# Allenxuxu/gev

Hardware: AMD Instinct MI355X
Metric: GiB/s WS payload unmasked (device-resident) + frames/s, 64 KiB masked frames (higher is better)
Workload: dtype u8

## Files before the change

gev_amd/csrc/gevws_walk.hip:

```cpp
#include <chrono>

#include "gevws_internal.hpp"
#include "gevws_small.hpp"

namespace {

__device__ __forceinline__ void put_partial(uint64_t* part, uint32_t b, int k, uint64_t v, uint32_t tag) {
  uint64_t* p = part + 2 * ((uint64_t)b * kDecFields + k);
  put_granule(p, (uint32_t)v, tag);
  put_granule(p + 1, (uint32_t)(v >> 32), tag);
}

__device__ void scan_partials_wave(const uint64_t* __restrict__ part, uint32_t tag, uint64_t* __restrict__ blk,
                                   uint32_t nblk, uint64_t max_frames, uint64_t payload_cap,
                                   gevws_summary* __restrict__ sum) {
  constexpr int P = 4;
  const int lane = threadIdx.x & 63;
  uint64_t carry[kDecFields] = {0, 0, 0, 0, 0};
  uint32_t bad = 0;
  for (uint64_t base = 0; base < nblk; base += 64 * P) {
    const uint64_t i0 = base + (uint64_t)lane * P;
    uint64_t g[P][kDecFields][2];
#pragma unroll
    for (int r = 0; r < P; ++r)
#pragma unroll
      for (int k = 0; k < kDecFields; ++k)
#pragma unroll
        for (int h = 0; h < 2; ++h)
          g[r][k][h] = (i0 + r < nblk) ? load_granule(part + 2 * ((i0 + r) * kDecFields + k) + h) : 0;
    uint64_t loc[kDecFields] = {0, 0, 0, 0, 0};
    uint64_t loc0[P], loc1[P];
#pragma unroll
    for (int r = 0; r < P; ++r)
#pragma unroll
      for (int k = 0; k < kDecFields; ++k) {
        uint64_t v = 0;
        if (i0 + r < nblk) {
          const uint64_t* q = part + 2 * ((i0 + r) * kDecFields + k);
          v = (uint64_t)take_granule(q, g[r][k][0], tag, bad) | ((uint64_t)take_granule(q + 1, g[r][k][1], tag, bad) << 32);
        }
        loc[k] += v;
        if (k == 0) loc0[r] = v;
        if (k == 1) loc1[r] = v;
      }
    const uint64_t inc0 = wave_incl_scan(loc[0]), inc1 = wave_incl_scan(loc[1]);
    uint64_t b0 = carry[0] + inc0 - loc[0], b1 = carry[1] + inc1 - loc[1];
#pragma unroll
    for (int r = 0; r < P; ++r) {
      if (i0 + r < nblk) {
        uint64_t* q = blk + (i0 + r) * kDecFields;
        q[0] = b0;
        q[1] = b1;
        b0 += loc0[r];
        b1 += loc1[r];
      }
    }
#pragma unroll
    for (int k = 0; k < kDecFields; ++k) carry[k] += wave_sum(loc[k]);
  }
  bad = (uint32_t)wave_sum(bad);
  if (lane == 0) {
    gevws_summary sm;
    memset(&sm, 0, sizeof(sm));
    sm.frames = carry[0];
    sm.payload_bytes = carry[1];
    sm.payload_len = carry[2];
    sm.errors = carry[3] & 0xffffffffull;
    sm.flags = (carry[3] >> 32) ? GEVWS_SUMMARY_UNORDERED : 0u;
    sm.run_frames = carry[4];
    sm.status = bad ? GEVWS_ERR_DEVICE
                    : (carry[0] > max_frames || carry[1] > payload_cap) ? GEVWS_ERR_CAPACITY : GEVWS_OK;
    *sum = sm;
  }
}

__device__ __forceinline__ void walk_block_done(uint32_t* __restrict__ done, uint32_t nblk, const uint64_t* __restrict__ part,
                                                uint32_t tag, uint64_t* __restrict__ blk, uint64_t max_frames,
                                                uint64_t payload_cap, gevws_summary* __restrict__ sum, bool wrote) {
  __shared__ uint32_t s_last;
  if (wrote) __builtin_amdgcn_s_waitcnt(0);
  __syncthreads();
  if (threadIdx.x == 0)
    s_last = __hip_atomic_fetch_add(done, 1u, __ATOMIC_RELAXED, __HIP_MEMORY_SCOPE_AGENT) == nblk - 1 ? 1u : 0u;
  __syncthreads();
  if (s_last) {
    if (threadIdx.x < 64) scan_partials_wave(part, tag, blk, nblk, max_frames, payload_cap, sum);
    if (threadIdx.x == 0) __hip_atomic_store(done, 0u, __ATOMIC_RELAXED, __HIP_MEMORY_SCOPE_AGENT);
  }
}

constexpr uint64_t kWriterChainsPerCU = 128;
constexpr uint32_t kEntryGranMinShift = 6;
constexpr uint64_t kEntryBudget = 1ull << 29;
constexpr uint32_t kSlotShift = 5;
constexpr uint64_t kSlotAlign = 1ull << kSlotShift;
constexpr uint32_t kLenEsc = (1u << 21) - 1;
struct WalkEntry {
  uint32_t mask;
  uint32_t w;
};
static_assert(sizeof(WalkEntry) == 8, "one dwordx2 per entry");
__device__ __forceinline__ WalkEntry make_entry(uint32_t key, uint64_t L, uint32_t meta) {
  const uint32_t hlen = meta >> 16, masked = (meta >> 8) & 1u;
  const uint32_t ext = hlen - 2 - 4 * masked;
  const uint32_t form = ext == 0 ? 0u : (ext == 2 ? 1u : 2u);
  const uint32_t l21 = L < kLenEsc ? (uint32_t)L : kLenEsc;
  return WalkEntry{key, (meta & 0x1ffu) | (form << 9) | (l21 << 11)};
}
__device__ __forceinline__ uint32_t entry_hlen(const WalkEntry& e) {
  const uint32_t form = (e.w >> 9) & 3u;
  return 2 + (form == 2 ? 8u : 2u * form) + 4 * ((e.w >> 8) & 1u);
}
__device__ __forceinline__ uint32_t entry_len21(const WalkEntry& e) { return e.w >> 11; }

__device__ __forceinline__ bool entry_slots_of(const gevws_conn_in& ci, uint32_t c, uint64_t n_entries,
                                              uint32_t gshift, uint64_t& base, uint64_t& cap) {
  if (n_entries == 0 || ci.len >= (1ull << 32)) return false;
  base = kSlotAlign * ((ci.off >> (gshift + kSlotShift)) + (uint64_t)c);
  cap = kSlotAlign * ((ci.len >> (gshift + kSlotShift)) + 1);
  return base + cap <= n_entries;
}

__device__ __forceinline__ bool out_of_order(const gevws_conn_in* __restrict__ conns, uint32_t c,
                                             const gevws_conn_in& ci) {
  if (c == 0) return false;
  const gevws_conn_in p = conns[c - 1];
  return ci.off < p.off || ci.off - p.off < p.len;
}

__device__ __forceinline__ int walk_parse(uint64_t lo, uint64_t hi, uint64_t avail, uint32_t& meta, uint32_t& hlen,
                                          uint64_t& L, uint32_t& key) {
  const uint32_t b1 = (uint32_t)(lo >> 8) & 0xffu;
  const uint32_t masked = b1 >> 7, len7 = b1 & 0x7fu;
  const bool e16 = len7 == 126, e64 = len7 == 127;
  hlen = 2 + (e64 ? 8u : (e16 ? 2u : 0u)) + 4 * masked;
  const uint64_t L64 = __builtin_bswap64((lo >> 16) | (hi << 48));
  const uint64_t L16 = (((lo >> 16) & 0xff) << 8) | ((lo >> 24) & 0xff);
  L = e64 ? L64 : (e16 ? L16 : (uint64_t)len7);
  key = (e64 ? (uint32_t)(hi >> 16) : (e16 ? (uint32_t)(lo >> 32) : (uint32_t)(lo >> 16))) & (0u - masked);
  meta = ((uint32_t)lo & 0xffu) | (masked << 8) | (hlen << 16);
  const bool have_hdr = avail >= 6 && avail >= hlen;
  if (have_hdr && e64 && (L64 >> 63)) return GEVWS_ERR_LEN_MSB;
  return (have_hdr && avail - hlen >= L) ? GEVWS_OK : GEVWS_NEED_MORE;
}

struct WalkRes {
  uint64_t pos, nf, pb, pl, same, lastf, firstf, err;
  int32_t st;
  bool rec;
};
__device__ __forceinline__ WalkRes walk_res_fresh(uint64_t err = 0, int32_t st = GEVWS_OK) {
  WalkRes R;
  R.pos = R.nf = R.pb = R.pl = R.same = R.firstf = 0;
// ... 95 lines not shown
            qhi[0] = nhi;
            bool stop = false;
#pragma unroll
            for (int j = 0; j < D; ++j) {
              if (!stop && (uint32_t)j < qn) {
                uint32_t m2, h2, k2;
                uint64_t L2;
                const int r = walk_parse(qlo[j], qhi[j], len - pos, m2, h2, L2, k2);
                if (r != GEVWS_OK) {
                  if (r == GEVWS_ERR_LEN_MSB) { st = GEVWS_ERR_LEN_MSB; err += 1; }
                  fail = stop = true;
                } else {
                  put_entry(k2, L2, m2);
                  pos += h2 + L2;
                  if (h2 + L2 != fsz) {
                    stop = true;
                    run = 1;
                    prev_fsz = h2 + L2;
                  }
                }
              }
            }
            if (fail) break;
            load_window(s + pos, nlo, nhi);
            if (stop || qn < (uint32_t)D || pos + fsz > len) break;
          }
          if (fail) return false;
          if constexpr (ST == 0) *sink = WalkEntry{0, 0};
        }
      }
      return true;
    };
    uint64_t lo2 = 0, hi2 = 0;
    for (;;) {
      if (!step(lo, hi, lo2, hi2)) break;
      if (!step(lo2, hi2, lo, hi)) break;
    }
    R.pos = pos;
    R.nf = nf;
    R.pb = pb;
    R.pl = pl;
    R.same = same;
    R.lastf = lastf;
    R.firstf = firstf;
    R.err = err;
    R.st = st;
    R.rec = rec;
    if constexpr (ST == 2) {
      __asm__ volatile("" ::: "memory");
      lds_st(ring.head, (uint32_t)nf | kRingDone);
    }
}

template <uint32_t GROUP = kWriterGroup, uint32_t RING = kRing>
__device__ __forceinline__ void walk_ring_writer(WalkEntry* __restrict__ entries, WalkRing ring, uint64_t ebase,
                                                 uint64_t ecap) {
  static_assert(GROUP <= kSlotAlign && kSlotAlign % GROUP == 0 && RING % GROUP == 0 && GROUP % 4 == 0,
                "groups aligned by the slot runs, whole groups in the ring");
  uint32_t t = 0;
  bool fin = false;
  for (;;) {
    if (!fin) {
      const uint32_t hv = lds_ld(ring.head);
      __asm__ volatile("" ::: "memory");
      const uint32_t h = hv & ~kRingDone;
      while (h - t >= GROUP) {
        WalkEntry g[GROUP];
#pragma unroll
        for (uint32_t k = 0; k < GROUP; ++k) g[k] = ring.e[(t + k) & (RING - 1)];
        if (ebase != ~0ull && t + GROUP <= ecap) {
          u32x4* d = reinterpret_cast<u32x4*>(entries + ebase + t);
#pragma unroll
          for (uint32_t k = 0; k < GROUP / 2; ++k)
            d[k] = u32x4{g[2 * k].mask, g[2 * k].w, g[2 * k + 1].mask, g[2 * k + 1].w};
        }
        t += GROUP;
        __asm__ volatile("" ::: "memory");
        lds_st(ring.tail, t);
      }
      if (hv & kRingDone) {
        for (; t < h; ++t)
          if (ebase != ~0ull && t < ecap) entries[ebase + t] = ring.e[t & (RING - 1)];
        fin = true;
      }
    }
    if (__all(fin)) break;
    __builtin_amdgcn_s_sleep(2);
  }
}

template <int D, int ST>
__global__ __launch_bounds__(ST == 2 ? 2 * kCountBlock : kCountBlock) void k_walk_count(
    const uint8_t* __restrict__ in, const gevws_conn_in* __restrict__ conns, uint32_t n,
    gevws_conn_out* __restrict__ cout, uint64_t* __restrict__ blk, WalkEntry* __restrict__ entries, uint64_t n_entries,
    uint32_t gshift, uint32_t cpb, uint64_t in_bytes, uint32_t* __restrict__ done, uint64_t* __restrict__ part,
    uint32_t tag, uint64_t max_frames, uint64_t payload_cap, gevws_summary* __restrict__ sum) {
  __shared__ WalkEntry s_ring[ST == 2 ? kCountBlock * kRing : 1];
  __shared__ uint32_t s_head[ST == 2 ? kCountBlock : 1], s_tail[ST == 2 ? kCountBlock : 1];
  __shared__ uint64_t s_ebase[ST == 2 ? kCountBlock : 1], s_ecap[ST == 2 ? kCountBlock : 1];
  const uint32_t lane = threadIdx.x & 63;
  const bool walker = ST != 2 || threadIdx.x < 64;
  const uint32_t c = blockIdx.x * cpb + lane;
  const bool active = walker && lane < cpb && c < n;
  uint64_t nf = 0, pb = 0, pl = 0, err = 0, same = 0;
  gevws_conn_in ci = {0, 0};
  int32_t st = GEVWS_OK;
  uint64_t ebase = 0, ecap = 0;
  bool rec0 = false;
  if (active) {
    ci = conns[c];
    if (out_of_order(conns, c, ci)) err = 1ull << 32;
    if (ci.off > in_bytes || ci.len > in_bytes - ci.off) {
      ci.off = 0;
      ci.len = 0;
      st = GEVWS_ERR_INVALID;
      err += 1;
    }
    rec0 = entry_slots_of(ci, c, n_entries, gshift, ebase, ecap);
  }
  const WalkRing ring = {s_ring + lane * kRing, s_head + lane, s_tail + lane};
  if constexpr (ST == 2) {
    if (walker) {
      s_head[lane] = active ? 0u : kRingDone;
      s_tail[lane] = 0;
      s_ebase[lane] = rec0 ? ebase : ~0ull;
      s_ecap[lane] = ecap;
    }
    __syncthreads();
    if (!walker) walk_ring_writer(entries, ring, s_ebase[lane], s_ecap[lane]);
  }
  if (active) {
    WalkRes R = walk_res_fresh(err, st);
    walk_chain<D, ST>(in + ci.off, ci.len, rec0, ebase, ecap, entries, entries + n_entries + c, R, ring);
    nf = R.nf;
    pb = R.pb;
    pl = R.pl;
    err = R.err;
    same = R.same;
    gevws_conn_out o;
    o.first_frame = R.rec ? 1 : 0;
    o.consumed = R.pos;
    o.payload_base = pb;
    o.nframes = (uint32_t)nf;
    o.status = R.st;
    cout[c] = o;
  }
  const uint64_t vals[kDecFields] = {nf, pb, pl, err, same};
#pragma unroll
  for (int k = 0; k < kDecFields; ++k) {
    const uint64_t s = wave_sum(vals[k]);
    if (threadIdx.x == 0) {
      if (done) put_partial(part, blockIdx.x, k, s, tag);
      else blk[(uint64_t)blockIdx.x * kDecFields + k] = s;
    }
  }
  if (done) walk_block_done(done, gridDim.x, part, tag, blk, max_frames, payload_cap, sum, threadIdx.x == 0);
}

constexpr uint32_t kSyncWin = 256;
constexpr uint32_t kSyncRow = kSyncWin / 4 + 5;
constexpr int kSyncDepth = 5;
constexpr uint32_t kSplitAutoMaxLanes = 16;
constexpr uint64_t kSplitMinFramesPerConn = 256;
constexpr uint64_t kSplitMaxConnsPerCU = 64;
constexpr uint64_t kSplitMaxFrameBytes = 4096;

__device__ __forceinline__ bool sync_plausible1(uint32_t b0, uint32_t b1, uint32_t m0) {
  const uint32_t op = b0 & 0x0fu;
  const bool data = op <= 2, ctrl = op >= 8 && op <= 10;
  return (b0 & 0x70u) == 0 && (b1 >> 7) == m0 && (data || (ctrl && (b0 & 0x80u) && (b1 & 0x7fu) <= 125));
}

__device__ __forceinline__ uint64_t sync_frame(uint64_t lo, uint64_t hi, uint64_t rem, uint32_t m0) {
  const uint32_t b0 = (uint32_t)lo & 0xffu, b1 = (uint32_t)(lo >> 8) & 0xffu;
  if (!sync_plausible1(b0, b1, m0)) return 0;
  const uint32_t len7 = b1 & 0x7fu;
  const uint32_t hlen = 2 + (len7 == 127 ? 8u : (len7 == 126 ? 2u : 0u)) + 4 * (b1 >> 7);
  uint64_t L = len7;
  if (len7 == 126) {
    L = (((lo >> 16) & 0xff) << 8) | ((lo >> 24) & 0xff);
    if (L < 126) return 0;
  } else if (len7 == 127) {
    L = __builtin_bswap64((lo >> 16) | (hi << 48));
    if ((L >> 63) || L < 65536) return 0;
  }
  if (rem < hlen || rem - hlen < L) return 0;
  return hlen + L;
}

__device__ __forceinline__ void row_window(const uint32_t* __restrict__ row, uint32_t x, uint64_t& lo, uint64_t& hi) {
  const uint32_t k = x >> 2, e = x & 3;
  const uint32_t w0 = row[k], w1 = row[k + 1], w2 = row[k + 2], w3 = row[k + 3], w4 = row[k + 4];
  lo = (uint64_t)__builtin_amdgcn_alignbyte(w1, w0, e) | ((uint64_t)__builtin_amdgcn_alignbyte(w2, w1, e) << 32);
  hi = (uint64_t)__builtin_amdgcn_alignbyte(w3, w2, e) | ((uint64_t)__builtin_amdgcn_alignbyte(w4, w3, e) << 32);
}

__device__ __forceinline__ uint32_t sync_l1_mask4(uint32_t w, uint32_t wn, uint32_t mpat) {
  const uint32_t w1 = __builtin_amdgcn_alignbyte(wn, w, 1);
  const uint32_t bad = (w & 0x74747474u) | (w & (w >> 1) & 0x01010101u) | ((w1 ^ mpat) & 0x80808080u);
  const uint32_t z = ~(((bad & 0x7f7f7f7fu) + 0x7f7f7f7fu) | bad | 0x7f7f7f7fu);
  return ((z >> 7) & 1u) | ((z >> 14) & 2u) | ((z >> 21) & 4u) | ((z >> 28) & 8u);
}

constexpr int kSyncWindows = 4;
constexpr int kSyncMinInWindow = 1;
__device__ __forceinline__ bool sync_search(const uint8_t* __restrict__ s, uint64_t len, uint64_t t, uint64_t step,
                                            uint64_t qmax, uint32_t m0, uint32_t* __restrict__ row, uint64_t& b) {
  const uint32_t mpat = m0 ? 0x80808080u : 0u;
  for (int win = 0; win < kSyncWindows; ++win, t += step) {
    if (t + kSyncWin + 16 > len || t >= qmax) return false;
    uint32_t wv[kSyncRow - 1];
#pragma unroll
    for (uint32_t j = 0; j < (kSyncWin + 16) / 16; ++j) {
      const u32x4 v = ld16u(s + t + 16 * j);
#pragma unroll
      for (int e = 0; e < 4; ++e) wv[4 * j + e] = v[e];
    }
#pragma unroll
    for (uint32_t k = 0; k < kSyncRow - 1; ++k) row[k] = wv[k];
    row[kSyncRow - 1] = 0;
    uint64_t cm[kSyncWin / 64];
#pragma unroll
    for (uint32_t j = 0; j < kSyncWin / 64; ++j) {
      uint64_t m = 0;
#pragma unroll
      for (uint32_t k = 0; k < 16; ++k) m |= (uint64_t)sync_l1_mask4(wv[16 * j + k], wv[16 * j + k + 1], mpat) << (4 * k);
      cm[j] = m;
    }
    bool have = false;
    uint64_t q = 0, lb = 0;
    int h = 0;
#pragma unroll
    for (uint32_t j = 0; j < kSyncWin / 64; ++j) {
      uint64_t m = have ? 0 : cm[j];
      while (m) {
        uint32_t x = 64 * j + (uint32_t)__builtin_ctzll(m);
        m &= m - 1;
        uint64_t lo, hi;
        row_window(row, x, lo, hi);
        uint64_t f = sync_frame(lo, hi, len - (t + x), m0);
        if (f == 0) continue;
        int hh = 1;
        uint32_t last = x;
        while (hh < kSyncDepth && x + f < kSyncWin) {
          x += (uint32_t)f;
          row_window(row, x, lo, hi);
          f = sync_frame(lo, hi, len - (t + x), m0);
          if (f == 0) break;
          last = x;
          ++hh;
        }
        if (f == 0 || (hh < kSyncMinInWindow && t + x + f < len)) continue;
        have = true;
        q = t + x + f;
        lb = t + last;
        h = hh;
        m = 0;
      }
    }
    if (!have) continue;
    bool ok = true;
    while (h < kSyncDepth) {
      if (q >= qmax || q >= len) {
        ok = false;
        break;
      }
      uint64_t lo, hi;
      load_window(s + q, lo, hi);
      const uint64_t g = sync_frame(lo, hi, len - q, m0);
      if (g == 0) {
        ok = false;
        break;
      }
      lb = q;
      q += g;
      ++h;
    }
    if (ok && lb < qmax) {
      b = lb;
      return true;
    }
  }
  return false;
}

constexpr uint32_t kSplitRing = 32;
constexpr uint32_t kSplitGroup = 16;
constexpr uint32_t kSplitLdsWords = (kCountBlock * kSyncRow > 2 * kCountBlock * kSplitRing)
                                        ? kCountBlock * kSyncRow
                                        : 2 * kCountBlock * kSplitRing;

template <int KS, int D, int ST>
__global__ __launch_bounds__(ST == 2 ? 2 * kCountBlock : kCountBlock) void k_walk_split(const uint8_t* __restrict__ in,
                                                            const gevws_conn_in* __restrict__ conns, uint32_t n,
                                                            gevws_conn_out* __restrict__ cout,
                                                            uint64_t* __restrict__ blk,
                                                            WalkEntry* __restrict__ entries, uint64_t n_entries,
                                                            uint32_t gshift, uint32_t cpb, uint64_t in_bytes,
                                                            uint32_t* __restrict__ done,
                                                            uint64_t* __restrict__ part, uint32_t tag,
                                                            uint64_t max_frames,
                                                            uint64_t payload_cap, gevws_summary* __restrict__ sum,
                                                            gevws_conn_in* __restrict__ segs,
                                                            gevws_conn_out* __restrict__ sout,
                                                            uint8_t* __restrict__ srec,
                                                            uint64_t min_seg = kSplitMinBytes,
// ... 393 lines not shown
        pbase = o.payload_base;
        coff = ci.off;
      }
      for (uint64_t m = __ballot(lane < GL && nf > 0); m; m &= m - 1) {
        const int j = __builtin_ctzll(m);
        const uint64_t cnt = uniform64(__shfl(nf, j, 64));
        const uint64_t fj = uniform64(__shfl(ff, j, 64)), pj = uniform64(__shfl(pbase, j, 64));
        const uint64_t oj = uniform64(__shfl(coff, j, 64)), ej = uniform64(__shfl(ebase, j, 64));
        one_conn(cnt, fj, pj, oj, ej);
      }
    }
  }
  const uint64_t nthreads = (uint64_t)gridDim.x * kWalkBlock;
  for (uint64_t c = (uint64_t)blockIdx.x * kWalkBlock + threadIdx.x; c < n; c += nthreads) {
    if (rec_flags[c] && !unordered) continue;
    const gevws_conn_out o = out_of(c);
    const gevws_conn_in ci = conns[c];
    const uint8_t* s = in + ci.off;
    uint64_t pos = 0, poff = o.payload_base;
    for (uint64_t k = 0; k < o.nframes; ++k) {
      uint64_t lo, hi;
      load_window(s + pos, lo, hi);
      DevHdr h;
      parse_header(lo, hi, ci.len - pos, h);
      emit_record(frames, tile_first, o.first_frame + k, poff, ci.off + pos + h.hlen, h);
      poff += round16(h.length);
      pos += h.hlen + h.length;
    }
  }
}

template <class S>
__global__ __launch_bounds__(S::NT) void k_decode_small(const uint8_t* __restrict__ in, uint64_t in_bytes,
                                                        const gevws_conn_in* __restrict__ conns, uint32_t n,
                                                        gevws_frame* __restrict__ frames, uint64_t max_frames,
                                                        uint8_t* __restrict__ payload, uint64_t payload_cap,
                                                        gevws_conn_out* __restrict__ cout,
                                                        gevws_summary* __restrict__ sum,
                                                        uint32_t* __restrict__ done = nullptr,
                                                        uint32_t seq = 0, uint64_t* __restrict__ ticks = nullptr,
                                                        uint64_t* __restrict__ stage_buf = nullptr,
                                                        uint32_t* __restrict__ stage_done = nullptr,
                                                        uint32_t tag = 0, uint64_t* __restrict__ phase = nullptr) {
  (void)decode_small_body<S>(in, in_bytes, conns, n, frames, max_frames, payload, payload_cap, cout, sum, done, seq,
                             ticks, stage_buf, stage_done, tag, gridDim.x, blockIdx.x, gridDim.x, phase);
}

template <class S>
__global__ __launch_bounds__(S::NT) void k_decode_small_direct(DirectDecodeArgs a) {
  (void)decode_small_body<S>(a.in, a.in_bytes, a.conns, a.n, a.frames, a.max_frames, a.payload, a.payload_cap,
                             a.cout, a.sum, a.done, a.seq, a.ticks, a.stage_buf, a.stage_done, a.tag, a.nwg,
                             blockIdx.x, a.nwg, a.phase);
}

constexpr uint32_t kServiceMaxPasses = 1u << 16;
constexpr uint32_t kSvcCmd = 0, kSvcSeq = 1, kSvcArgs = 2, kSvcExit = kSvcArgs + 2 * kServiceArgs,
                   kSvcDone = kSvcExit + 1, kSvcCtlGranules = kSvcDone + 1;

template <class S>
__global__ __launch_bounds__(S::NT) void k_decode_service(ServiceBox* __restrict__ box, uint32_t gen, uint32_t req0,
                                                          uint64_t life_ticks, uint32_t* __restrict__ done,
                                                          uint64_t* __restrict__ ticks, uint64_t* __restrict__ ctl,
                                                          uint64_t* __restrict__ stage_buf,
                                                          uint32_t* __restrict__ stage_done, uint32_t t0) {
  __shared__ uint32_t s_k, s_slices, s_req;
  __shared__ uint64_t s_a[kServiceArgs];
  const uint64_t t_start = gpu_ticks();
  const uint32_t wg = blockIdx.x, G = gridDim.x;
  uint32_t last = req0;
  uint32_t k = 0;
  for (;;) {
    if (threadIdx.x == 0) {
      uint32_t slices = 0, req = 0;
      if (wg == 0) {
        while (k + 1 < kServiceMaxPasses) {
          const uint64_t w = __hip_atomic_load(&box->req, __ATOMIC_ACQUIRE, __HIP_MEMORY_SCOPE_SYSTEM);
          if ((uint32_t)(w >> 32) == gen && (uint32_t)w != last) {
            last = req = (uint32_t)w;
            break;
          }
          if (__hip_atomic_load(&box->gen, __ATOMIC_RELAXED, __HIP_MEMORY_SCOPE_SYSTEM) != gen ||
              gpu_ticks() - t_start >= life_ticks)
            break;
          __builtin_amdgcn_s_sleep(2);
        }
        if (req) {
          const uint32_t tag = t0 + ++k;
          for (int i = 0; i < kServiceArgs; ++i)
            s_a[i] = __hip_atomic_load(&box->args[i], __ATOMIC_RELAXED, __HIP_MEMORY_SCOPE_SYSTEM);
          __hip_atomic_store(&box->ack, req, __ATOMIC_RELEASE, __HIP_MEMORY_SCOPE_SYSTEM);
          slices = small_slices(s_a[1], (uint32_t)s_a[3], G);
          if (slices > 1) {
            for (int i = 0; i < kServiceArgs; ++i) {
              put_granule(ctl + kSvcArgs + 2 * i, (uint32_t)s_a[i], tag);
              put_granule(ctl + kSvcArgs + 2 * i + 1, (uint32_t)(s_a[i] >> 32), tag);
            }
            put_granule(ctl + kSvcSeq, req, tag);
          }
          put_granule(ctl + kSvcCmd, slices, tag);
        } else {
          if (k)
            for (uint64_t t1 = gpu_ticks(); (uint32_t)(load_granule(ctl + kSvcDone) >> 32) != t0 + k &&
                                            gpu_ticks() - t1 < life_ticks;)
              __builtin_amdgcn_s_sleep(2);
          put_granule(ctl + kSvcExit, 0u, t0);
        }
      } else {
        for (;;) {
          const uint64_t g = load_granule(ctl + kSvcCmd);
          const uint32_t d = (uint32_t)(g >> 32) - t0;
          if (d > k && d < kServiceMaxPasses) {
            k = d;
            if ((uint32_t)g > wg) {
              slices = (uint32_t)g;
              break;
            }
            continue;
          }
          if ((uint32_t)(load_granule(ctl + kSvcExit) >> 32) == t0 || gpu_ticks() - t_start >= 2 * life_ticks) break;
          __builtin_amdgcn_s_sleep(2);
        }
        uint32_t bad = 0;
        const uint32_t tag = t0 + k;
        for (int i = 0; slices && i < kServiceArgs; ++i) {
          const uint64_t* p = ctl + kSvcArgs + 2 * i;
          const uint32_t lo = take_granule(p, load_granule(p), tag, bad);
          const uint32_t hi = take_granule(p + 1, load_granule(p + 1), tag, bad);
          s_a[i] = (uint64_t)lo | ((uint64_t)hi << 32);
        }
        if (slices) req = take_granule(ctl + kSvcSeq, load_granule(ctl + kSvcSeq), tag, bad);
        if (bad) slices = 0;
      }
      s_k = k;
      s_slices = slices;
      s_req = req;
    }
    __syncthreads();
    const uint32_t slices = s_slices;
    if (!slices) return;
    __builtin_amdgcn_fence(__ATOMIC_ACQUIRE, "");
    const uint32_t tag = t0 + s_k;
    const bool decoded = decode_small_body<S>(
        reinterpret_cast<const uint8_t*>(s_a[0]), s_a[1], reinterpret_cast<const gevws_conn_in*>(s_a[2]),
        (uint32_t)s_a[3], reinterpret_cast<gevws_frame*>(s_a[4]), s_a[5], reinterpret_cast<uint8_t*>(s_a[6]), s_a[7],
        reinterpret_cast<gevws_conn_out*>(s_a[8]), reinterpret_cast<gevws_summary*>(s_a[9]), done, s_req, ticks,
        stage_buf, stage_done, tag, slices, wg, slices);
    if (decoded && threadIdx.x == 0) put_granule(ctl + kSvcDone, 0u, tag);
    __syncthreads();
  }
}

const char* const kWalkVariants[] = {
    "default: one lane per connection with uniform-stream speculation (D = 8; plain D = 0 after a batch of mixed "
    "sizes on this context); from 128 connections per CU the entries go through an LDS ring to a writer wave "
    "(256-byte groups); the split walk for few long chains of small frames",
    "one lane per connection, plain chain walk (D = 0)",
    "no entry table (the record pass re-walks every chain)",
    "entries through the writer wave whatever the batch size (the default's path for >= 128 connections per CU)",
    "the default, with the split walk's entries stored by the walking lanes (no writer wave; measurement)",
};
constexpr int kNumWalkVariants = sizeof(kWalkVariants) / sizeof(kWalkVariants[0]);

}

namespace gevws_impl {

int walk_variant_count() { return kNumWalkVariants; }
const void* direct_kernel_stub(int wide) {
  return wide ? reinterpret_cast<const void*>(&k_decode_small_direct<SmallWide>)
              : reinterpret_cast<const void*>(&k_decode_small_direct<SmallNarrow>);
}
uint32_t split_fallback_counter() { return kSplitFallbackCounter; }
const char* walk_variant_name(int i) { return i >= 0 && i < kNumWalkVariants ? kWalkVariants[i] : nullptr; }

static uint64_t* phase_ticks(const gevws_ctx* ctx) {
  static const bool on = [] {
    const char* e = getenv("GEVWS_PHASE_TICKS");
    return e && e[0] == '1';
  }();
  return on && ctx->done_flag && ctx->ticks ? ctx->ticks + 2 : nullptr;
}

template <class S>
static int launch_decode_small(gevws_ctx* ctx, hipStream_t st, const uint8_t* d_in, uint64_t in_bytes,
                               const gevws_conn_in* d_conns, uint32_t n_conns, gevws_frame* d_frames,
                               uint64_t max_frames, uint8_t* d_payload, uint64_t payload_cap,
                               gevws_conn_out* d_conn_out, gevws_summary* d_summary) {
  const uint32_t seq = ctx->done_flag ? ++ctx->done_seq : 0u;
  uint32_t nwg = 1;
  if (ctx->done_flag && n_conns) {
    nwg = small_slices(in_bytes, n_conns, kSmallStageWGs);
    if (nwg > 1 && !ensure_small_stage(ctx, st)) nwg = 1;
  }
  const uint32_t tag = nwg > 1 ? next_hand_tag(ctx) : 0u;
  k_decode_small<S><<<nwg, S::NT, 0, st>>>(d_in, in_bytes, d_conns, n_conns, d_frames, max_frames, d_payload,
                                           payload_cap, d_conn_out, d_summary, ctx->done_flag, seq,
                                           ctx->done_flag ? ctx->ticks : nullptr, ctx->d_small_stage,
                                           ctx->d_done + kSmallStageCounter, tag, phase_ticks(ctx));
  GEVWS_HIP(hipGetLastError());
  const int r = ctx->prev_small_decode ? mark_last_lazy(ctx, st) : mark_last(ctx, st);
  ctx->prev_small_decode = true;
  if (ctx->done_flag) ctx->last_signal = seq;
  return r;
}

constexpr uint64_t kServiceLifeMs = 200;
constexpr int64_t kServiceUseMs = 100;

static int64_t host_ns() {
  return std::chrono::duration_cast<std::chrono::nanoseconds>(std::chrono::steady_clock::now().time_since_epoch())
      .count();
}

bool service_post(gevws_ctx* ctx, hipStream_t st, const uint8_t* d_in, uint64_t in_bytes,
                  const gevws_conn_in* d_conns, uint32_t n_conns, gevws_frame* d_frames, uint64_t max_frames,
                  uint8_t* d_payload, uint64_t payload_cap, gevws_conn_out* d_conn_out, gevws_summary* d_summary) {
  if (!ctx->svc_enabled || !ctx->svc_box || !ctx->done_flag || st != ctx->stream || n_conns > kSmallConns ||
      in_bytes > kSmallBytes)
    return false;
  if (__atomic_load_n(&ctx->svc_box->ack, __ATOMIC_ACQUIRE) != ctx->svc_last) return false;
  const int64_t now = host_ns();
  if (ctx->svc_live) {
    if (now - ctx->svc_t_launch_ns > kServiceUseMs * 1000000 || ctx->svc_flag != ctx->done_flag ||
        ctx->svc_ticks != ctx->ticks || ctx->svc_passes + 2 >= kServiceMaxPasses)
      service_stop(ctx);
    else if ((int32_t)(__atomic_load_n(ctx->svc_flag_host, __ATOMIC_ACQUIRE) - ctx->svc_last) < 0)
      return false;
  }
  if (!ctx->svc_live) {
    if (ctx->last_direct) {
      if (direct_drain(ctx) != GEVWS_OK) return false;
      ctx->last_direct = false;
    }
    hipPointerAttribute_t pa;
    if (hipPointerGetAttributes(&pa, ctx->done_flag) != hipSuccess || !pa.hostPointer) return false;
    if (!ensure_small_stage(ctx, st)) return false;
    if (!ctx->d_svc_ctl) {
      const size_t cb = kSvcCtlGranules * sizeof(uint64_t);
      if (hipMalloc(reinterpret_cast<void**>(&ctx->d_svc_ctl), cb) != hipSuccess) {
        ctx->d_svc_ctl = nullptr;
        return false;
      }
      if (hipMemsetAsync(ctx->d_svc_ctl, 0, cb, st) != hipSuccess) return false;
    }
    if (ctx->has_last && ctx->last_stream != st &&
        (last_event(ctx) != GEVWS_OK || hipStreamWaitEvent(st, ctx->last_done, 0) != hipSuccess))
      return false;
    const uint32_t gen = ++ctx->svc_gen;
    const uint32_t t0 = reserve_hand_tags(ctx, kServiceMaxPasses);
    __atomic_store_n(&ctx->svc_box->gen, gen, __ATOMIC_RELEASE);
    k_decode_service<SmallNarrow><<<kSmallStageWGs, SmallNarrow::NT, 0, st>>>(
        ctx->svc_box_dev, gen, ctx->svc_last, kServiceLifeMs * ctx->wall_khz, ctx->done_flag, ctx->ticks,
        ctx->d_svc_ctl, ctx->d_small_stage, ctx->d_done + kSmallStageCounter, t0);
    if (hipGetLastError() != hipSuccess || mark_last_lazy(ctx, st) != GEVWS_OK) {
      __atomic_store_n(&ctx->svc_box->gen, ++ctx->svc_gen, __ATOMIC_RELEASE);
      return false;
    }
    ctx->svc_live = true;
    ctx->svc_t_launch_ns = now;
    ctx->svc_flag = ctx->done_flag;
    ctx->svc_flag_host = static_cast<const uint32_t*>(pa.hostPointer);
    ctx->svc_ticks = ctx->ticks;
    ctx->svc_t0 = t0;
    ctx->svc_passes = 0;
    ++ctx->svc_launches;
  }
  uint32_t seq = ++ctx->done_seq;
  if (seq == 0) seq = ++ctx->done_seq;
  const uint64_t a[kServiceArgs] = {reinterpret_cast<uint64_t>(d_in),      in_bytes,
                                    reinterpret_cast<uint64_t>(d_conns),   n_conns,
                                    reinterpret_cast<uint64_t>(d_frames),  max_frames,
                                    reinterpret_cast<uint64_t>(d_payload), payload_cap,
                                    reinterpret_cast<uint64_t>(d_conn_out), reinterpret_cast<uint64_t>(d_summary)};
  for (int k = 0; k < kServiceArgs; ++k) __atomic_store_n(&ctx->svc_box->args[k], a[k], __ATOMIC_RELAXED);
  __atomic_store_n(&ctx->svc_box->req, ((uint64_t)ctx->svc_gen << 32) | seq, __ATOMIC_RELEASE);
  ctx->svc_last = seq;
  ctx->last_signal = seq;
  ++ctx->svc_passes;
  ++ctx->svc_posts;
  return true;
}

int decode_small(gevws_ctx* ctx, hipStream_t st, const uint8_t* d_in, uint64_t in_bytes,
                 const gevws_conn_in* d_conns, uint32_t n_conns, gevws_frame* d_frames, uint64_t max_frames,
                 uint8_t* d_payload, uint64_t payload_cap, gevws_conn_out* d_conn_out, gevws_summary* d_summary) {
  if (n_conns > kOneLaunchConns || in_bytes > kOneLaunchBytes) return GEVWS_ERR_INVALID;
  const int r = order_after_last(ctx, st);
  if (r != GEVWS_OK) return r;
  if (n_conns <= kSmallConns && in_bytes <= kSmallBytes)
    return launch_decode_small<SmallNarrow>(ctx, st, d_in, in_bytes, d_conns, n_conns, d_frames, max_frames,
                                            d_payload, payload_cap, d_conn_out, d_summary);
  return launch_decode_small<SmallWide>(ctx, st, d_in, in_bytes, d_conns, n_conns, d_frames, max_frames, d_payload,
                                        payload_cap, d_conn_out, d_summary);
}

bool direct_post(gevws_ctx* ctx, const uint8_t* d_in, uint64_t in_bytes, const gevws_conn_in* d_conns,
                 uint32_t n_conns, gevws_frame* d_frames, uint64_t max_frames, uint8_t* d_payload,
                 uint64_t payload_cap, gevws_conn_out* d_conn_out, gevws_summary* d_summary) {
  if (!ctx->direct_enabled || !ctx->done_flag || n_conns > kOneLaunchConns || in_bytes > kOneLaunchBytes)
    return false;
  service_stop(ctx);
  const int wide = n_conns <= kSmallConns && in_bytes <= kSmallBytes ? 0 : 1;
  uint32_t nwg = n_conns ? small_slices(in_bytes, n_conns, kSmallStageWGs) : 1u;
  if (nwg > 1 && !ctx->d_small_stage) {
    if (!ensure_small_stage(ctx, ctx->stream)) nwg = 1;
    else if (hipStreamSynchronize(ctx->stream) != hipSuccess) return false;
  }
  DirectDecodeArgs a;
  a.in = d_in;
  a.in_bytes = in_bytes;
  a.conns = d_conns;
  a.frames = d_frames;
  a.max_frames = max_frames;
  a.payload = d_payload;
  a.payload_cap = payload_cap;
  a.cout = d_conn_out;
  a.sum = d_summary;
  a.done = ctx->done_flag;
  a.ticks = ctx->ticks;
  a.stage_buf = ctx->d_small_stage;
  a.stage_done = ctx->d_done + kSmallStageCounter;
  a.n = n_conns;
  uint32_t seq = ctx->done_seq + 1;
  if (seq == 0) seq = 1;
  a.seq = seq;
  a.tag = nwg > 1 ? next_hand_tag(ctx) : 0u;
  a.nwg = nwg;
  a.phase = phase_ticks(ctx);
  if (!direct_dispatch(ctx, wide, a)) return false;
  ctx->done_seq = seq;
  ctx->last_signal = seq;
  return true;
}

int decode_front(gevws_ctx* ctx, hipStream_t st, const uint8_t* d_in, uint64_t in_bytes,
                 const gevws_conn_in* d_conns, uint32_t n_conns, gevws_frame* d_frames, uint64_t max_frames,
                 uint64_t payload_cap, gevws_conn_out* d_conn_out, gevws_summary* d_summary, hipEvent_t* ev,
                 uint32_t** tile_first_out) {
  const uint32_t ncu = (uint32_t)ctx->num_cus;
  const uint32_t cpb = n_conns >= (uint32_t)kCountBlock * ncu ? (uint32_t)kCountBlock
                                                             : (n_conns + ncu - 1) / ncu > 0 ? (n_conns + ncu - 1) / ncu : 1;
  if (ctx->stats_pending && hipEventQuery(ctx->last_done) == hipSuccess) {
    ctx->stats_pending = false;
    ctx->stats_known = true;
    const uint64_t fr = ctx->h_stats[0], pl = ctx->h_stats[1];
    ctx->prev_frames_per_conn = ctx->stats_conns ? fr / ctx->stats_conns : 0;
    ctx->prev_frame_bytes = fr ? pl / fr : 0;
    ctx->prev_mixed = 2 * ctx->h_stats[2] < fr;
  }
  const int wv = ctx->walk_variant;
  uint32_t ks = 1;
  if ((wv == 0 || wv == 4) && n_conns) {
    if (ctx->split_lanes >= 2) {
      ks = ctx->split_lanes;
    } else if (ctx->split_lanes == 0 && in_bytes / n_conns >= 2 * kSplitMinBytes && ctx->stats_known &&
               ctx->prev_frames_per_conn >= kSplitMinFramesPerConn && ctx->prev_frame_bytes <= kSplitMaxFrameBytes) {
      if ((uint64_t)n_conns <= kSplitMaxConnsPerCU * ncu)
        while (ks < kSplitAutoMaxLanes && (uint64_t)n_conns * ks * 2 <= ctx->split_lanes_per_cu * ncu) ks *= 2;
    }
  }
  if ((uint64_t)n_conns * ks > 0xFFFFFFFFull) ks = 1;
  ctx->last_ks = ks;
  const uint32_t cpb_w = ks > 1 ? (kCountBlock / ks < cpb ? kCountBlock / ks : cpb) : cpb;
  const uint32_t nblk = (n_conns + cpb_w - 1) / cpb_w;
  const uint64_t n_v = (uint64_t)n_conns * ks;
  const uint64_t ntiles_cap = (payload_cap + kTile - 1) / kTile + 1;
  const size_t blk_bytes = ((size_t)nblk * kDecFields * sizeof(uint64_t) + 255) & ~size_t(255);
  const size_t tile_bytes = (ntiles_cap * sizeof(uint32_t) + 255) & ~size_t(255);
  uint32_t gshift = kEntryGranMinShift;
  while ((in_bytes >> gshift) > kEntryBudget) ++gshift;
  const uint64_t n_entries = kSlotAlign * ((in_bytes >> (gshift + kSlotShift)) + n_v + 1);
  const size_t flag_bytes = ((size_t)n_conns + 255) & ~size_t(255);
  const size_t seg_bytes = ks > 1 ? ((n_v * (sizeof(gevws_conn_in) + sizeof(gevws_conn_out) + 1) + 1023) & ~size_t(255)) : 0;
  int r = order_after_last(ctx, st);
  if (r != GEVWS_OK) return r;
  const size_t run_bytes = kUnmaskRunCounters * 64;
  r = ensure_scratch(ctx, blk_bytes + tile_bytes + run_bytes + flag_bytes + seg_bytes +
                              (n_entries + n_v) * sizeof(WalkEntry));
  if (r != GEVWS_OK) return r;
  char* sp = reinterpret_cast<char*>(ctx->scratch);
  uint64_t* blk = reinterpret_cast<uint64_t*>(sp);
  uint32_t* tile_first = reinterpret_cast<uint32_t*>(sp + blk_bytes);
  ctx->unmask_runs = reinterpret_cast<uint32_t*>(sp + blk_bytes + tile_bytes);
  uint8_t* rec_flags = reinterpret_cast<uint8_t*>(sp + blk_bytes + tile_bytes + run_bytes);
  char* segp = sp + blk_bytes + tile_bytes + run_bytes + flag_bytes;
  gevws_conn_in* segs = reinterpret_cast<gevws_conn_in*>(segp);
  gevws_conn_out* sout = reinterpret_cast<gevws_conn_out*>(segp + n_v * sizeof(gevws_conn_in));
  uint8_t* srec = reinterpret_cast<uint8_t*>(segp + n_v * (sizeof(gevws_conn_in) + sizeof(gevws_conn_out)));
  WalkEntry* entries = reinterpret_cast<WalkEntry*>(segp + seg_bytes);
  *tile_first_out = tile_first;
  if (ev) GEVWS_HIP(hipEventRecord(ev[0], st));
  const uint64_t ne = wv == 2 ? 0 : n_entries;
  const bool fused = nblk > 0 && nblk <= kFusedScanMaxBlocks;
  constexpr int kDecScanBlock = 256;
  uint32_t* done = fused ? ctx->d_done : nullptr;
  const uint32_t tag = fused ? next_hand_tag(ctx) : 0u;
  const bool plain = wv == 1 || (wv != 1 && ctx->stats_known && ctx->prev_mixed);
  if (nblk && ks > 1) {
    const bool writer = wv != 4;
    GEVWS_HIP(hipMemsetAsync(ctx->d_done + kSplitFallbackCounter, 0, sizeof(uint32_t), st));
#define GEVWS_SPLIT(K)                                                                                            \
  (writer ? (plain ? k_walk_split<K, 0, 2> : k_walk_split<K, 8, 2>)                                               \
          : (plain ? k_walk_split<K, 0, 0> : k_walk_split<K, 8, 0>))<<<nblk, writer ? 2 * kCountBlock : kCountBlock, \
                                                                      0, st>>>(                                     \
      d_in, d_conns, n_conns, d_conn_out, blk, entries, ne, gshift, cpb_w, in_bytes, done, ctx->d_walk_part, tag,     \
      max_frames, payload_cap,                                                                                      \
      d_summary, segs, sout, srec, ctx->split_min_bytes, ctx->d_done + kSplitFallbackCounter)
    if (ks == 2) GEVWS_SPLIT(2);
    else if (ks == 4) GEVWS_SPLIT(4);
    else if (ks == 8) GEVWS_SPLIT(8);
    else if (ks == 16) GEVWS_SPLIT(16);
    else GEVWS_SPLIT(32);
#undef GEVWS_SPLIT
  } else if (nblk && (wv == 3 || (uint64_t)n_conns >= kWriterChainsPerCU * (uint64_t)ncu)) {
    (plain ? k_walk_count<0, 2> : k_walk_count<8, 2>)<<<nblk, 2 * kCountBlock, 0, st>>>(
        d_in, d_conns, n_conns, d_conn_out, blk, entries, ne, gshift, cpb, in_bytes, done, ctx->d_walk_part, tag,
        max_frames, payload_cap, d_summary);
  } else if (nblk) {
    (plain ? k_walk_count<0, 0> : k_walk_count<8, 0>)<<<nblk, kCountBlock, 0, st>>>(
        d_in, d_conns, n_conns, d_conn_out, blk, entries, ne, gshift, cpb, in_bytes, done, ctx->d_walk_part, tag,
        max_frames, payload_cap, d_summary);
  }
  if (ev) GEVWS_HIP(hipEventRecord(ev[1], st));
  if (!fused) k_scan_blocks<true, kDecFields, kDecScanBlock><<<1, kDecScanBlock, 0, st>>>(blk, nblk, max_frames, payload_cap,
                                                                                         d_summary);
  if (ev) GEVWS_HIP(hipEventRecord(ev[2], st));
  if (nblk) {
    k_walk_bases<<<nblk, kCountBlock, 0, st>>>(n_conns, d_conn_out, blk, d_summary, rec_flags, cpb_w, ctx->d_stats,
                                               ctx->unmask_runs);
    ctx->stats_pending = true;
    ctx->stats_conns = n_conns;
    const gevws_conn_in* e_conns = ks > 1 ? segs : d_conns;
    const gevws_conn_out* e_out = ks > 1 ? sout : d_conn_out;
    const uint8_t* e_rec = ks > 1 ? srec : rec_flags;
    const gevws_conn_out* e_parent = ks > 1 ? d_conn_out : nullptr;
    uint64_t egrid = (n_v + kWalkBlock / 64 - 1) / (kWalkBlock / 64);
    const uint64_t ecap = (ks > 1 ? kEmitSplitPerCU : 8) * (uint64_t)ncu;
    if (egrid > ecap) egrid = ecap;
    k_walk_emit<<<(uint32_t)egrid, kWalkBlock, 0, st>>>(d_in, e_conns, (uint32_t)n_v, e_out, d_summary, d_frames,
                                                          tile_first, entries, ne, gshift, e_rec, e_parent,
                                                          ks > 1 ? ks : 0);
  }
  GEVWS_HIP(hipGetLastError());
  return GEVWS_OK;
}

}
```

Before: 2901.

## Walk each connection with a whole wave when connections per CU are few

Adds a k_walk_wave kernel that gives each connection a full 64-lane wave. Once three equal-sized frames appear in a row, the wave speculatively parses 64 frames at once using a ballot and prefix checks. It is chosen by default for non-plain, non-split batches with at most 16 connections per CU (tunable by an environment variable). The goal is to remove the serial per-lane chain walk when there are too few connections to fill the GPU. The cost is idle lanes on mixed-size streams and an extra per-block LDS reduction.

```diff
diff --git a/gev_amd/csrc/gevws_walk.hip b/gev_amd/csrc/gevws_walk.hip
--- a/gev_amd/csrc/gevws_walk.hip
+++ b/gev_amd/csrc/gevws_walk.hip
@@ -1,4 +1,5 @@
 #include <chrono>
+#include <cstdlib>
 
 #include "gevws_internal.hpp"
 #include "gevws_small.hpp"
@@ -400,6 +401,123 @@
     if (threadIdx.x == 0) {
       if (done) put_partial(part, blockIdx.x, k, s, tag);
       else blk[(uint64_t)blockIdx.x * kDecFields + k] = s;
+    }
+  }
+  if (done) walk_block_done(done, gridDim.x, part, tag, blk, max_frames, payload_cap, sum, threadIdx.x == 0);
+}
+
+constexpr uint32_t kWaveWalkWaves = 16;
+constexpr uint64_t kWaveWalkMaxConnsPerCU = kWaveWalkWaves;
+
+__global__ __launch_bounds__(64 * kWaveWalkWaves) void k_walk_wave(
+    const uint8_t* __restrict__ in, const gevws_conn_in* __restrict__ conns, uint32_t n,
+    gevws_conn_out* __restrict__ cout, uint64_t* __restrict__ blk, WalkEntry* __restrict__ entries, uint64_t n_entries,
+    uint32_t gshift, uint32_t cpb, uint64_t in_bytes, uint32_t* __restrict__ done, uint64_t* __restrict__ part,
+    uint32_t tag, uint64_t max_frames, uint64_t payload_cap, gevws_summary* __restrict__ sum) {
+  __shared__ uint64_t s_vals[kWaveWalkWaves][kDecFields];
+  const uint32_t lane = threadIdx.x & 63, wave = threadIdx.x >> 6, nwaves = blockDim.x >> 6;
+  uint64_t t_nf = 0, t_pb = 0, t_pl = 0, t_err = 0, t_same = 0;
+  for (uint32_t j = wave; j < cpb; j += nwaves) {
+    const uint32_t c = blockIdx.x * cpb + j;
+    if (c >= n) break;
+    gevws_conn_in ci = conns[c];
+    uint64_t err = out_of_order(conns, c, ci) ? 1ull << 32 : 0;
+    int32_t st = GEVWS_OK;
+    if (ci.off > in_bytes || ci.len > in_bytes - ci.off) {
+      ci.off = 0;
+      ci.len = 0;
+      st = GEVWS_ERR_INVALID;
+      err += 1;
+    }
+    uint64_t ebase = 0, ecap = 0;
+    bool rec = entry_slots_of(ci, c, n_entries, gshift, ebase, ecap);
+    const uint8_t* s = in + ci.off;
+    const uint64_t len = ci.len;
+    WalkEntry* const sink = entries + n_entries + c;
+    uint64_t pos = 0, nf = 0, pb = 0, pl = 0, same = 0, lastf = ~0ull, prev_fsz = 0;
+    uint32_t run = 0;
+    uint64_t lo, hi;
+    load_window(s, lo, hi);
+    for (;;) {
+      uint32_t meta, hlen, key;
+      uint64_t L;
+      const int r = walk_parse(lo, hi, len - pos, meta, hlen, L, key);
+      if (r != GEVWS_OK) {
+        if (r == GEVWS_ERR_LEN_MSB) {
+          st = GEVWS_ERR_LEN_MSB;
+          err += 1;
+        }
+        break;
+      }
+      const uint64_t fsz = (uint64_t)hlen + L;
+      pos += fsz;
+      run = fsz == prev_fsz ? run + 1 : 1;
+      prev_fsz = fsz;
+      if (run < 3) load_window(s + pos, lo, hi);
+      rec = rec && nf < ecap;
+      *((rec && lane == 0) ? entries + ebase + nf : sink) = make_entry(key, L, meta);
+      ++nf;
+      pb += round16(L);
+      pl += L;
+      same += fsz == lastf;
+      lastf = fsz;
+      if (run < 3) continue;
+      for (;;) {
+        const uint64_t q = pos + (uint64_t)lane * fsz;
+        const bool inside = q <= len;
+        uint64_t qlo, qhi;
+        load_window(s + (inside ? q : len), qlo, qhi);
+        uint32_t m2, h2, k2;
+        uint64_t L2;
+        const int r2 = walk_parse(qlo, qhi, inside ? len - q : 0, m2, h2, L2, k2);
+        const bool okf = inside && r2 == GEVWS_OK && (uint64_t)h2 + L2 == fsz;
+        const uint64_t bad = ~__ballot(okf);
+        const uint32_t p = bad ? (uint32_t)__builtin_ctzll(bad) : 64u;
+        const bool mine = lane < p;
+        if (mine && rec && nf + lane < ecap) entries[ebase + nf + lane] = make_entry(k2, L2, m2);
+        rec = rec && (p == 0 || nf + p <= ecap);
+        pb += wave_sum(mine ? round16(L2) : 0);
+        pl += wave_sum(mine ? L2 : 0);
+        nf += p;
+        same += p;
+        pos += (uint64_t)p * fsz;
+        if (p < 64) {
+          lo = __shfl(qlo, (int)p, 64);
+          hi = __shfl(qhi, (int)p, 64);
+          break;
+        }
+      }
+    }
+    if (lane == 0) {
+      gevws_conn_out o;
+      o.first_frame = rec ? 1 : 0;
+      o.consumed = pos;
+      o.payload_base = pb;
+      o.nframes = (uint32_t)nf;
+      o.status = st;
+      cout[c] = o;
+    }
+    t_nf += nf;
+    t_pb += pb;
+    t_pl += pl;
+    t_err += err;
+    t_same += same;
+  }
+  if (lane == 0) {
+    s_vals[wave][0] = t_nf;
+    s_vals[wave][1] = t_pb;
+    s_vals[wave][2] = t_pl;
+    s_vals[wave][3] = t_err;
+    s_vals[wave][4] = t_same;
+  }
+  __syncthreads();
+  if (threadIdx.x == 0) {
+#pragma unroll
+    for (int k = 0; k < kDecFields; ++k) {
+      uint64_t x = 0;
+      for (uint32_t w = 0; w < nwaves; ++w) x += s_vals[w][k];
+      if (done) put_partial(part, blockIdx.x, k, x, tag);
+      else blk[(uint64_t)blockIdx.x * kDecFields + k] = x;
     }
   }
   if (done) walk_block_done(done, gridDim.x, part, tag, blk, max_frames, payload_cap, sum, threadIdx.x == 0);
@@ -1099,12 +1217,13 @@
 
 const char* const kWalkVariants[] = {
     "default: one lane per connection with uniform-stream speculation (D = 8; plain D = 0 after a batch of mixed "
-    "sizes on this context); from 128 connections per CU the entries go through an LDS ring to a writer wave "
+    "sizes on this context), a wave per connection (64 frames a round) for few connections; from 128 connections per CU the entries go through an LDS ring to a writer wave "
     "(256-byte groups); the split walk for few long chains of small frames",
     "one lane per connection, plain chain walk (D = 0)",
     "no entry table (the record pass re-walks every chain)",
     "entries through the writer wave whatever the batch size (the default's path for >= 128 connections per CU)",
-    "the default, with the split walk's entries stored by the walking lanes (no writer wave; measurement)",
+    "the default, with the split walk's entries stored by the walking lanes (no writer wave) and the lane walk's "
+    "D = 8 speculation where the default gives a connection a wave (measurement)",
 };
 constexpr int kNumWalkVariants = sizeof(kWalkVariants) / sizeof(kWalkVariants[0]);
 
@@ -1126,6 +1245,14 @@
     return e && e[0] == '1';
   }();
   return on && ctx->done_flag && ctx->ticks ? ctx->ticks + 2 : nullptr;
+}
+
+static uint64_t wave_walk_max_conns_per_cu() {
+  static const uint64_t v = [] {
+    const char* e = getenv("GEVWS_WAVE_WALK_CONNS_PER_CU");
+    return e && e[0] ? (uint64_t)strtoull(e, nullptr, 10) : kWaveWalkMaxConnsPerCU;
+  }();
+  return v;
 }
 
 template <class S>
@@ -1343,6 +1470,7 @@
   uint32_t* done = fused ? ctx->d_done : nullptr;
   const uint32_t tag = fused ? next_hand_tag(ctx) : 0u;
   const bool plain = wv == 1 || (wv != 1 && ctx->stats_known && ctx->prev_mixed);
+  const bool wave_walk = wv == 0 && ks == 1 && !plain && (uint64_t)n_conns <= wave_walk_max_conns_per_cu() * ncu;
   if (nblk && ks > 1) {
     const bool writer = wv != 4;
     GEVWS_HIP(hipMemsetAsync(ctx->d_done + kSplitFallbackCounter, 0, sizeof(uint32_t), st));
@@ -1359,6 +1487,10 @@
     else if (ks == 16) GEVWS_SPLIT(16);
     else GEVWS_SPLIT(32);
 #undef GEVWS_SPLIT
+  } else if (nblk && wave_walk) {
+    const uint32_t nw = cpb < kWaveWalkWaves ? cpb : kWaveWalkWaves;
+    k_walk_wave<<<nblk, 64 * nw, 0, st>>>(d_in, d_conns, n_conns, d_conn_out, blk, entries, ne, gshift, cpb, in_bytes,
+                                          done, ctx->d_walk_part, tag, max_frames, payload_cap, d_summary);
   } else if (nblk && (wv == 3 || (uint64_t)n_conns >= kWriterChainsPerCU * (uint64_t)ncu)) {
     (plain ? k_walk_count<0, 2> : k_walk_count<8, 2>)<<<nblk, 2 * kCountBlock, 0, st>>>(
         d_in, d_conns, n_conns, d_conn_out, blk, entries, ne, gshift, cpb, in_bytes, done, ctx->d_walk_part, tag,
```

Result: slower. 2442 (-15.8%).
